# damaggu/StableKeypoints

Measured on AMD Instinct MI355X. Metric: images/sec (token-opt step, 512², N=500 tokens), higher is better.
Workload: dtype f32

## Files before the change

### include/skp.h

```cpp
#ifndef SKP_H
#define SKP_H

#ifdef __cplusplus
extern "C" {
#endif

#define SKP_OK 0
#define SKP_EBADARG (-1)
#define SKP_ELAUNCH (-2)
#define SKP_MAX_LAYERS 16

const char* skp_last_error(void);
int skp_version(void);

int skp_capture_fwd(const float* z_low, int BH, int s, int N, int R, float* attn, float* stats, void* stream);

int skp_capture_bwd(const float* z_low, int BH, int s, int N, int R, const float* dattn, int group, long long sb,
                    long long sp, long long sn, float gscale, const float* stats, float* dz_low, float* workspace,
                    void* stream);

int skp_capture_maps_fwd(const float* const* z_low, const int* sizes, int L, int B, int H, int N, int R, float* maps,
                         float* const* stats, void* stream);

int skp_capture_maps_bwd(const float* const* z_low, const int* sizes, int L, int B, int H, int N, int R,
// ... 133 lines not shown
int skp_wino2_weights(const float* w, int K, int C, int flip, float* U, void* stream);
int skp_conv3x3_wino2(const float* x, const float* U, const float* bias, const float* residual, float* y, int B,
                      int C, int K, int H, int W, int nsplit, float* ws, void* stream);
int skp_conv3x3_wino2_gn(const float* x, const float* U, const float* bias, const float* residual, float* y, int B,
                         int C, int K, int H, int W, int nsplit, float* ws, float* gn_part, void* stream);
int skp_wino2_vtransform(const float* x, float* V, int B, int C, int H, int W, void* stream);
int skp_wino2_vtransform_gn(const float* x, const float* stats, const float* gamma, const float* beta,
                            const float* shift, int G, int act, float* V, int B, int C, int H, int W, void* stream);
int skp_conv3x3_wino2_v(const float* V, const float* U, const float* bias, const float* residual, float* y, int B,
                        int C, int K, int H, int W, int nsplit, float* ws, void* stream);
int skp_conv3x3_wino2_v_gn(const float* V, const float* U, const float* bias, const float* residual, float* y, int B,
                           int C, int K, int H, int W, int nsplit, float* ws, float* gn_part, void* stream);
int skp_wino2s2_weights(const float* w, int K, int C, float* U, void* stream);
int skp_conv3x3s2_f2(const float* x, const float* U, const float* bias, float* y, int B, int C, int K, int H, int W,
                     int nsplit, float* ws, void* stream);

int skp_map_range(const float* maps, int n, int h, int w, float* range, void* stream);
int skp_render_sheet(const float* images, int n, int H, int W, const float* maps, int h, int w, const float* range,
                     const float* lut, float alpha, const float* points, int K, float radius,
                     const unsigned char* colors, int rows, int cols, int f, int pad, unsigned char* out,
                     void* stream);

int skp_tta_reduce_workspace(int B, int n, int S);
int skp_tta_reduce(const float* maps, int B, int C, int n, int S, const float* theta_inv, float* pos, float* avg,
                   void* workspace, void* stream);

#ifdef __cplusplus
}
#endif
#endif
// ... 1 lines not shown
```

### stablekeypoints_amd/_lib.py

```python
import ctypes
import os

import torch

_HERE = os.path.dirname(os.path.abspath(__file__))
LIB_PATH = os.environ.get("SKP_LIB", os.path.join(_HERE, "libskp.so"))

_c_int, _c_float, _c_ll, _p = ctypes.c_int, ctypes.c_float, ctypes.c_longlong, ctypes.c_void_p

_SIGS = {
    "skp_capture_fwd": [_p, _c_int, _c_int, _c_int, _c_int, _p, _p, _p],
    "skp_capture_bwd": [_p, _c_int, _c_int, _c_int, _c_int, _p, _c_int, _c_ll, _c_ll, _c_ll, _c_float, _p, _p, _p,
                        _p],
    "skp_capture_maps_fwd": [ctypes.POINTER(_p), ctypes.POINTER(_c_int), _c_int, _c_int, _c_int, _c_int, _c_int, _p,
                             ctypes.POINTER(_p), _p],
    "skp_capture_maps_bwd": [ctypes.POINTER(_p), ctypes.POINTER(_c_int), _c_int, _c_int, _c_int, _c_int, _c_int, _p,
                             _c_float, ctypes.POINTER(_p), ctypes.POINTER(_p), _p, _p],
    "skp_capture_maps_bwd_sel": [ctypes.POINTER(_p), ctypes.POINTER(_c_int), _c_int, _c_int, _c_int, _c_int, _c_int,
                                 _p, _c_int, _p, _c_float, ctypes.POINTER(_p), ctypes.POINTER(_p), _p, _p],
    "skp_sel_bwd_timing": [_c_int],
    "skp_sel_bwd_timing_read": [_p, _p],
    "skp_capture_maps_bwd_sel_workspace": [ctypes.POINTER(_c_int), _c_int, _c_int, _c_int, _c_int, _c_int, _c_int],
    "skp_aggregate": [ctypes.POINTER(_p), _c_int, _c_int, _c_int, _c_int, _p, _c_int, _p, _p],
    "skp_resize_bilinear": [_p, _c_int, _c_int, _c_int, _p, _p],
# ... 52 lines not shown
    "skp_wino_weights": [_p, _c_int, _c_int, _c_int, _p, _p],
    "skp_conv3x3_wino": [_p, _p, _p, _p, _p, _c_int, _c_int, _c_int, _c_int, _c_int, _c_int, _p, _p],
    "skp_wino2_weights": [_p, _c_int, _c_int, _c_int, _p, _p],
    "skp_conv3x3_wino2": [_p, _p, _p, _p, _p, _c_int, _c_int, _c_int, _c_int, _c_int, _c_int, _p, _p],
    "skp_conv3x3_wino2_gn": [_p, _p, _p, _p, _p, _c_int, _c_int, _c_int, _c_int, _c_int, _c_int, _p, _p, _p],
    "skp_groupnorm_fwd_part": [_p, _p, _p, _p, _p, _c_int, _c_int, _c_int, _c_ll, _c_int, _c_float, _c_int, _p, _p, _p,
                               _p],
    "skp_groupnorm_stats": [_p, _p, _c_int, _c_int, _c_ll, _c_int, _c_float, _p, _p, _p],
    "skp_groupnorm_stats_part": [_p, _c_int, _p, _c_int, _c_int, _c_ll, _c_int, _c_float, _p, _p, _p],
    "skp_wino2_vtransform": [_p, _p, _c_int, _c_int, _c_int, _c_int, _p],
    "skp_wino2_vtransform_gn": [_p, _p, _p, _p, _p, _c_int, _c_int, _p, _c_int, _c_int, _c_int, _c_int, _p],
    "skp_conv3x3_wino2_v": [_p, _p, _p, _p, _p, _c_int, _c_int, _c_int, _c_int, _c_int, _c_int, _p, _p],
    "skp_conv3x3_wino2_v_gn": [_p, _p, _p, _p, _p, _c_int, _c_int, _c_int, _c_int, _c_int, _c_int, _p, _p, _p],
    "skp_wino2s2_weights": [_p, _c_int, _c_int, _p, _p],
    "skp_conv3x3s2_f2":   [_p, _p, _p, _p, _c_int, _c_int, _c_int, _c_int, _c_int, _c_int, _p, _p],
    "skp_map_range": [_p, _c_int, _c_int, _c_int, _p, _p],
    "skp_render_sheet": [_p, _c_int, _c_int, _c_int, _p, _c_int, _c_int, _p, _p, _c_float, _p, _c_int, _c_float, _p,
                         _c_int, _c_int, _c_int, _c_int, _p, _p],
    "skp_tta_reduce_workspace": [_c_int, _c_int, _c_int],
    "skp_tta_reduce": [_p, _c_int, _c_int, _c_int, _c_int, _p, _p, _p, _p, _p],
    "skp_version": [],
}


_RESTYPE = {"skp_capture_maps_bwd_sel_workspace": _c_ll}
_MEASUREMENT_ONLY = {"skp_sel_bwd_timing", "skp_sel_bwd_timing_read"}


class SkpLibraryError(RuntimeError):
    pass


_lib = None


def lib():
    global _lib
    if _lib is None:
        if not os.path.exists(LIB_PATH):
            raise SkpLibraryError(f"libskp.so not found at {LIB_PATH}: build it with "
                                  "`python -c 'import __graft_entry__ as g; g.build()'` or `make -C stablekeypoints_amd/csrc`")
# ... 41 lines not shown
```

### stablekeypoints_amd/csrc/skp_conv.hip

```cpp
#include <cstdlib>

#include "skp_common.h"
#include "skp_gn.h"

using namespace skp;

#ifndef SKP_WINO_DEBUG
#define SKP_WINO_DEBUG 0
#endif
#ifndef SKP_WINO2_DEBUG
#define SKP_WINO2_DEBUG 0
#endif

namespace {

typedef float f32x4 __attribute__((ext_vector_type(4)));
typedef unsigned int u32x4 __attribute__((ext_vector_type(4)));

constexpr int kMT = 64;
constexpr int kNC = 32;
constexpr int kCK = 4;
constexpr int kP = 36;
constexpr int kThreads = 512;
constexpr int kUs = kCK * kNC * kP;
// ... 625 lines not shown
    case 9: W2_VMCNT(9); break;
    case 10: W2_VMCNT(10); break;
    case 11: W2_VMCNT(11); break;
    case 12: W2_VMCNT(12); break;
    case 13: W2_VMCNT(13); break;
    case 14: W2_VMCNT(14); break;
    case 15: W2_VMCNT(15); break;
    default: W2_VMCNT(0); break;
  }
}

#ifndef SKP_W2_RS4
#define SKP_W2_RS4 0
#endif

template <int EPI, int HH, int TXB, int NW, bool VST = false, bool S2 = false>
__device__ __forceinline__ void wino2_body(const W2Smem& sm, const float* __restrict__ x, const float* __restrict__ U,
                                           const float* __restrict__ bias, const float* __restrict__ res,
                                           float* __restrict__ y, int C, int K, int H, int W, int img, int x0,
                                           int y0, int kb, int c0, int csplit, int wv, int dbg,
                                           float2* __restrict__ gnp) {
  using Geo = w2::GeoT<TXB, NW>;
  constexpr int kChF = Geo::CHF, kRowF = Geo::RF, kRawInstr = Geo::RAW_INSTR, NI = Geo::NI, RR = Geo::RR,
                RC = Geo::RC;
  static_assert(!S2 || (TXB == 8 && NW == 4 && !VST && (EPI & ~1) == 0), "stride-2 form: half-height blocks, bias only");
  constexpr int kUP = S2 ? w2::kUP2 : w2::kUP, kUF = S2 ? w2::kUF2 : w2::kUF, kUInstr = kUF / 256;
  constexpr int NP = S2 ? (HH ? 10 : 15) : 18;
  constexpr int kInstr = kRawInstr + kUInstr;
  constexpr int kMaxRaw = (kRawInstr + NW - 1) / NW;
  constexpr int kMaxU = (kUInstr + NW - 1) / NW + 1;
  constexpr int NT = NW * WAVE;
// ... 196 lines not shown
      }
    }

  }

  W2_VMCNT(0);
  __syncthreads();
  if (dbg & 32) return;
  if constexpr (S2) {
    constexpr int PLS2 = 8 * 16 + 4;
    static_assert(16 * PLS2 <= Geo::RAWF, "stride-2 exchange planes fit one raw slot");
    const int Ho = H / 2, Wo = W / 2;
    float* pl = R0 + (lane & 15) * PLS2 + 2 * (2 * wm + (lane >> 5)) * 16 + 8 * ((lane >> 4) & 1);
#pragma unroll
    for (int blk = 0; blk < 2; ++blk) {
      float o[4][4];
#pragma unroll
      for (int r = 0; r < 4; ++r) {
        float m[NP];
#pragma unroll
        for (int q = 0; q < NP; ++q) m[q] = acc[blk][q][r];
        w2::s2_output<HH>(m, o[r]);
      }
      if (HH != blk) {
#pragma unroll
        for (int f = 0; f < 2; ++f)
#pragma unroll
          for (int h = 0; h < 2; ++h)
            *reinterpret_cast<float4*>(pl + f * 16 + 4 * h) =
                make_float4(o[2 * h][2 * f], o[2 * h][2 * f + 1], o[2 * h + 1][2 * f], o[2 * h + 1][2 * f + 1]);
      }
      __syncthreads();
      if (HH == blk) {
#pragma unroll
        for (int f = 0; f < 2; ++f)
#pragma unroll
          for (int h = 0; h < 2; ++h) {
            float4* d = reinterpret_cast<float4*>(pl + f * 16 + 4 * h);
            const float4 p = *d;
            *d = make_float4(o[2 * h][2 * f] + p.x, o[2 * h][2 * f + 1] + p.y, o[2 * h + 1][2 * f] + p.z,
                             o[2 * h + 1][2 * f + 1] + p.w);
          }
      }
      __syncthreads();
#pragma unroll
      for (int i = 0; i < 16 * 32 / NT; ++i) {
        const int idx = i * NT + tid;
        const int c = idx >> 5, row = (idx >> 2) & 7, c4 = idx & 3;
        const float4 p = *reinterpret_cast<const float4*>(R0 + c * PLS2 + row * 16 + 4 * c4);
        const int k = kb * w2::kNC + 16 * blk + c;
        const float bv = (EPI & 1) ? bias[k] : 0.0f;
        const size_t o4 = (((size_t)img * K + k) * Ho + y0 / 2 + row) * Wo + x0 / 2 + 4 * c4;
        const float4 v = make_float4(p.x + bv, p.y + bv, p.z + bv, p.w + bv);
        if (dbg & 128) __builtin_nontemporal_store(f32x4{v.x, v.y, v.z, v.w}, reinterpret_cast<f32x4*>(y + o4));
        else if (!(dbg & 64)) *reinterpret_cast<float4*>(y + o4) = v;
      }
      if (blk == 0) __syncthreads();
    }
  } else {
    constexpr int PH = (TXB == 8 && NW == 4) ? 16 : 32;
    constexpr int PLS = (TXB == 8 ? PH * 32 : NI * 256) + 4;
    float* const P2 = RS == 2 ? U1 : R2;
    auto plane_of = [&](int c) -> float* {
      float* b = (c >> 2) == 0 ? R0 : (c >> 2) == 1 ? R1 : (c >> 2) == 2 ? P2 : U0;
      return b + (c & 3) * PLS + (c >> 2) * 16;
    };
    float* pl = plane_of(lane & 15);
    const int pbase = TXB == 8 ? (4 * (2 * wm + (lane >> 5))) * 32 + 4 * (4 * ((lane >> 4) & 1))
                               : wm * 256 + (4 * (lane >> 4)) * 16;
    constexpr int PW = TXB == 8 ? 32 : 16;
#pragma unroll
    for (int blk = 0; blk < 2; ++blk) {
      if (HH != blk) {
#pragma unroll
        for (int r = 0; r < 4; ++r) {
          float m[18], o[16];
#pragma unroll
          for (int q = 0; q < 18; ++q) m[q] = acc[blk][q][r];
          w2::half_output<HH>(m, o);
#pragma unroll
          for (int f = 0; f < 4; ++f)
            *reinterpret_cast<float4*>(pl + pbase + f * PW + 4 * r) =
                make_float4(o[4 * f], o[4 * f + 1], o[4 * f + 2], o[4 * f + 3]);
        }
      }
      __syncthreads();
      if (HH == blk) {
#pragma unroll
        for (int r = 0; r < 4; ++r) {
          float m[18], o[16];
#pragma unroll
          for (int q = 0; q < 18; ++q) m[q] = acc[blk][q][r];
          w2::half_output<HH>(m, o);
#pragma unroll
          for (int f = 0; f < 4; ++f) {
            float4* d = reinterpret_cast<float4*>(pl + pbase + f * PW + 4 * r);
            const float4 p = *d;
            *d = make_float4(o[4 * f] + p.x, o[4 * f + 1] + p.y, o[4 * f + 2] + p.z, o[4 * f + 3] + p.w);
          }
        }
      }
      __syncthreads();
      constexpr int PCF = TXB == 8 ? PH * 8 : NI * 64;
      constexpr int NIT = 16 * PCF / NT;
      static_assert(TXB != 8 || NIT == 8, "TXB 8: eight wave instructions per wave");
      float g1[4] = {0.f, 0.f, 0.f, 0.f}, g2[4] = {0.f, 0.f, 0.f, 0.f}, piv[4] = {0.f, 0.f, 0.f, 0.f};
#pragma unroll
      for (int i = 0; i < NIT; ++i) {
        const int idx = TXB == 8 ? (((tid >> 6) * NIT + i) << 6) + (tid & 63) : i * NT + tid;
        const int c = idx / PCF, q = idx % PCF;
        const float4 v0 = *reinterpret_cast<const float4*>(plane_of(c) + 4 * q);
        const int k = kb * w2::kNC + 16 * blk + c;
        const float bv = (EPI & 1) ? bias[k] : 0.0f;
        size_t o;
        if (TXB == 8) {
          const int row = q >> 3, c4 = q & 7;
          o = (((size_t)img * K + k) * H + y0 + row) * W + x0 + 4 * c4;
        } else {
          o = ((size_t)(img + (q >> 6)) * K + k) * 256 + 4 * (q & 63);
        }
        float4 v = make_float4(v0.x + bv, v0.y + bv, v0.z + bv, v0.w + bv);
        if (EPI & 2) {
          const float4 rv = *reinterpret_cast<const float4*>(res + o);
          v.x += rv.x;
          v.y += rv.y;
          v.z += rv.z;
          v.w += rv.w;
        }
        if (dbg & 128) __builtin_nontemporal_store(f32x4{v.x, v.y, v.z, v.w}, reinterpret_cast<f32x4*>(y + o));
        else if (!(dbg & 64)) *reinterpret_cast<float4*>(y + o) = v;
        if (TXB == 8 && gnp) {
          if ((i & 1) == 0) piv[i >> 1] = __builtin_bit_cast(float, __builtin_amdgcn_readfirstlane(__builtin_bit_cast(int, v.x)));
          const float p = piv[i >> 1];
          const float dx = v.x - p, dy = v.y - p, dz = v.z - p, dw = v.w - p;
          g1[i >> 1] += (dx + dy) + (dz + dw);
          g2[i >> 1] += (dx * dx + dy * dy) + (dz * dz + dw * dw);
        }
      }
// ... 25 lines not shown
          const int J = (tid >> 6) * NIT + 2 * r;
          const int c = (J << 6) / PCF, piece = ((J << 6) % PCF) >> 6;
          const int k = kb * w2::kNC + 16 * blk + c;
          const int seg = ((y0 + 8 * piece) >> 4) * (W >> 5) + (x0 >> 5);
          const float p = r == 0 ? piv[0] : r == 1 ? piv[1] : r == 2 ? piv[2] : piv[3];
          constexpr float inv_n = 1.0f / 512.0f;
          gnp[((size_t)img * K + k) * (size_t)((H >> 4) * (W >> 5)) + seg] =
              make_float2(p + x * inv_n, fmaxf(x2 - x * (x * inv_n), 0.0f));
        }
      }
      if (blk == 0) __syncthreads();
    }
  }
}

template <int EPI, int TXB, int NW = 8, bool S2 = false>
__global__ __launch_bounds__(NW * WAVE) __attribute__((amdgpu_waves_per_eu(2, 2))) void wino2_kernel(
    const float* __restrict__ x, const float* __restrict__ U, const float* __restrict__ bias,
    const float* __restrict__ res, float* __restrict__ y, int nimg, int C, int K, int H, int W, int bw, int bpi,
    int nblk, int nkb, int kb_major, int csplit, int dbg, float2* __restrict__ gnp) {
  __shared__ __attribute__((aligned(16))) float R0[w2::GeoT<TXB, NW>::RAWF], R1[w2::GeoT<TXB, NW>::RAWF],
      R2[(TXB == 4 && NW == 4) ? 4 : w2::GeoT<TXB, NW>::RAWF],
      R3[(TXB == 8 && NW == 8 && SKP_W2_RS4) ? w2::GeoT<TXB, NW>::RAWF : 4];
  constexpr int UF = S2 ? w2::kUF2 : w2::kUF;
  __shared__ __attribute__((aligned(16))) float U0[UF], U1[UF], U2[NW == 4 ? 4 : UF];
  const int G = gridDim.x;
  const int g = blockIdx.x;
  const int Lg = (G % 8 == 0) ? (g % 8) * (G / 8) + g / 8 : g;
  const int sp = Lg / (nblk * nkb);
  const int L = Lg - sp * (nblk * nkb);
  y += (size_t)sp * nimg * K * (S2 ? (H / 2) * (W / 2) : H * W);
  int tb, kb;
  if (kb_major) {
    kb = L / nblk;
    tb = L - kb * nblk;
  } else {
    tb = L / nkb;
    kb = L - tb * nkb;
  }
  int img, x0 = 0, y0 = 0;
  if (TXB == 8) {
    img = tb / bpi;
    const int br = tb - img * bpi;
    const int by = br / bw;
    x0 = 32 * (br - by * bw);
    y0 = (NW == 4 ? 16 : 32) * by;
  } else {
    img = (NW == 4 ? 2 : 4) * tb;
  }
  const int wv = __builtin_amdgcn_readfirstlane(threadIdx.x >> 6);
  const W2Smem sm{R0, R1, R2, R3, U0, U1, U2};
  const int c0 = sp * csplit;
  if (wv < NW / 2)
    wino2_body<EPI, 0, TXB, NW, false, S2>(sm, x, U, bias, res, y, C, K, H, W, img, x0, y0, kb, c0, csplit, wv, dbg, gnp);
  else wino2_body<EPI, 1, TXB, NW, false, S2>(sm, x, U, bias, res, y, C, K, H, W, img, x0, y0, kb, c0, csplit, wv, dbg, gnp);
}

__global__ void wino2_weights_kernel(const float* __restrict__ w, int K, int C, int flip, float* __restrict__ U) {
  const long long i = blockIdx.x * (long long)blockDim.x + threadIdx.x;
  if (i >= (long long)K * C) return;
  const int k = (int)(i / C), c = (int)(i - (long long)k * C);
  double g[9];
  for (int u = 0; u < 3; ++u)
    for (int v = 0; v < 3; ++v)
      g[3 * u + v] = flip ? (double)w[((size_t)c * K + k) * 9 + (2 - u) * 3 + (2 - v)]
                          : (double)w[((size_t)k * C + c) * 9 + u * 3 + v];
  const double Gm[6][3] = {{1.0, 0.0, 0.0},
                           {1.0 / 3, 1.0 / 3, 1.0 / 3},
                           {-1.0 / 3, 1.0 / 3, -1.0 / 3},
                           {-16.0 / 15, -8.0 / 15, -4.0 / 15},
// ... 18 lines not shown
  double g[9];
  for (int u = 0; u < 9; ++u) g[u] = (double)w[((size_t)k * C + c) * 9 + u];
  const double Gm[5][3] = {{1.0, 0.0, 0.0}, {1.0, 0.0, 1.0}, {0.0, 0.0, 1.0}, {0.0, 1.0, 0.0}, {0.0, 1.0, 0.0}};
  double t[5][3];
  for (int a = 0; a < 5; ++a)
    for (int v = 0; v < 3; ++v) t[a][v] = Gm[a][0] * g[v] + Gm[a][1] * g[3 + v] + Gm[a][2] * g[6 + v];
  float* out = U + (((size_t)(k / w2::kNC) * C + c) * w2::kNC + (k % w2::kNC)) * w2::kUP2;
  for (int p = 0; p < w2::kUP2; ++p) out[p] = 0.0f;
  for (int a = 0; a < 5; ++a)
    for (int b = 0; b < 5; ++b) {
      const int p = 5 * a + b;
      out[p < 15 ? p : p + 1] = (float)(t[a][0] * Gm[b][0] + t[a][1] * Gm[b][1] + t[a][2] * Gm[b][2]);
    }
}

template <int EPI>
__global__ __launch_bounds__(4 * WAVE) __attribute__((amdgpu_waves_per_eu(2, 2))) void wino2v_kernel(
    const float* __restrict__ V, const float* __restrict__ U, const float* __restrict__ bias,
    const float* __restrict__ res, float* __restrict__ y, int nimg, int C, int K, int H, int W, int bw, int bpi,
    int nblk, int nkb, int kb_major, int csplit, int dbg, float2* __restrict__ gnp) {
  __shared__ __attribute__((aligned(16))) float U0[w2::kUF], U1[w2::kUF], U2[w2::kUF];
  static_assert(3 * w2::kUF * 4 <= 80 * 1024, "two workgroups per CU");
  static_assert(4 * (16 * 32 + 4) + 48 <= w2::kUF / 2, "a plane buffer per half U slot");
  const int G = gridDim.x;
  const int g = blockIdx.x;
  const int Lg = (G % 8 == 0) ? (g % 8) * (G / 8) + g / 8 : g;
  const int sp = Lg / (nblk * nkb);
  const int L = Lg - sp * (nblk * nkb);
  y += (size_t)sp * nimg * K * H * W;
  int tb, kb;
  if (kb_major) {
    kb = L / nblk;
    tb = L - kb * nblk;
  } else {
    tb = L / nkb;
    kb = L - tb * nkb;
  }
  const int img = tb / bpi;
  const int br = tb - img * bpi;
  const int by = br / bw;
  const int x0 = 32 * (br - by * bw), y0 = 16 * by;
  const int wv = __builtin_amdgcn_readfirstlane(threadIdx.x >> 6);
  const W2Smem sm{U0 + w2::kUF / 2, U1 + w2::kUF / 2, nullptr, nullptr, U0, U1, U2};
  const int c0 = sp * csplit;
  if (wv < 2)
    wino2_body<EPI, 0, 8, 4, true>(sm, V, U, bias, res, y, C, K, H, W, img, x0, y0, kb, c0, csplit, wv, dbg, gnp);
  else wino2_body<EPI, 1, 8, 4, true>(sm, V, U, bias, res, y, C, K, H, W, img, x0, y0, kb, c0, csplit, wv, dbg, gnp);
}

template <int GN>
__global__ __launch_bounds__(4 * WAVE) void wino2_vtransform_kernel(
    const float* __restrict__ x, const float* __restrict__ stats, const float* __restrict__ gamma,
    const float* __restrict__ beta, const float* __restrict__ shift, int G, float* __restrict__ V, int C, int H, int W,
    int bw, int bpi) {
  using Geo = w2::GeoT<8, 4>;
  constexpr int RR = Geo::RR, RC = Geo::RC, kChF = Geo::CHF, kRowF = Geo::RF;
  __shared__ __attribute__((aligned(16))) float R[Geo::RAWF];
  const int tid = threadIdx.x, lane = tid & 63;
  const int nst = C / w2::kCK;
  const int tb = blockIdx.x / nst, st = blockIdx.x - tb * nst;
  const int img = tb / bpi;
  const int br = tb - img * bpi;
// ... 50 lines not shown
  SKP_CHECK_ARG(w && U, "null pointer");
  SKP_CHECK_ARG(K > 0 && C > 0, "non-positive shape");
  SKP_CHECK_ARG(K % w2::kNC == 0, "output channels must be a multiple of 32");
  const long long n = (long long)K * C;
  hipLaunchKernelGGL(wino2s2_weights_kernel, dim3((unsigned)((n + 255) / 256)), dim3(256), 0, as_stream(stream), w, K,
                     C, U);
  SKP_LAUNCH_CHECK();
  return SKP_OK;
}

namespace {
int wino_nt_flag(long long out_bytes, int nsplit) {
  if (nsplit > 1) return 0;
  return out_bytes >= (256LL << 20) ? 128 : 0;
}
}

extern "C" int skp_conv3x3s2_f2(const float* x, const float* U, const float* bias, float* y, int B, int C, int K,
                                int H, int W, int nsplit, float* ws, void* stream) {
  SKP_CHECK_ARG(x && U && y, "null pointer");
  SKP_CHECK_ARG(B > 0 && C > 0 && K > 0 && H > 0 && W > 0, "non-positive shape");
  SKP_CHECK_ARG(C % w2::kCK == 0, "input channels must be a multiple of 4");
  SKP_CHECK_ARG(K % w2::kNC == 0, "output channels must be a multiple of 32");
  SKP_CHECK_ARG(H % 32 == 0 && W % 32 == 0, "H and W must be multiples of 32");
  SKP_CHECK_ARG(nsplit >= 1 && C % (w2::kCK * nsplit) == 0, "nsplit must divide C into multiples of 4");
  SKP_CHECK_ARG(nsplit == 1 || ws, "split-K needs a workspace of nsplit·B·K·(H/2)·(W/2) floats");
  SKP_CHECK_ARG(aligned16(x) && aligned16(U) && aligned16(y) && (!ws || aligned16(ws)), "tensors must be 16-byte aligned");
  SKP_CHECK_ARG((long long)B * C * H * W * 4 < 0x7fffffffLL, "input larger than 2 GiB (32-bit buffer offsets)");
  const int bw = W / 32, bpi = (H / 16) * bw;
  const long long nblk = (long long)B * bpi;
  const int nkb = K / w2::kNC;
  SKP_CHECK_ARG(nblk * nkb * nsplit <= 0x7fffffffLL, "grid too large");
  float* out = nsplit > 1 ? ws : y;
  hipStream_t st = as_stream(stream);
  const dim3 grid((unsigned)(nblk * nkb * nsplit));
  const int fl = SKP_WINO2_DEBUG | wino_nt_flag((long long)B * K * (H / 2) * (W / 2) * 4, nsplit);
  if (nsplit == 1 && bias)
    hipLaunchKernelGGL((wino2_kernel<1, 8, 4, true>), grid, dim3(4 * WAVE), 0, st, x, U, bias, nullptr, out, B, C, K, H,
                       W, bw, bpi, (int)nblk, nkb, 0, C / nsplit, fl, nullptr);
  else
    hipLaunchKernelGGL((wino2_kernel<0, 8, 4, true>), grid, dim3(4 * WAVE), 0, st, x, U, nullptr, nullptr, out, B, C, K,
                       H, W, bw, bpi, (int)nblk, nkb, 0, C / nsplit, fl, nullptr);
  SKP_LAUNCH_CHECK();
  if (nsplit > 1) return splitk_reduce(ws, nsplit, B, K, (H / 2) * (W / 2), bias, nullptr, y, st);
  return SKP_OK;
}

extern "C" int skp_conv3x3_wino2_gn(const float* x, const float* U, const float* bias, const float* residual, float* y,
                                    int B, int C, int K, int H, int W, int nsplit, float* ws, float* gn_part,
                                    void* stream) {
  SKP_CHECK_ARG(x && U && y, "null pointer");
  SKP_CHECK_ARG(!gn_part || (nsplit == 1 && H % 32 == 0 && W % 32 == 0 && (reinterpret_cast<uintptr_t>(gn_part) & 7) == 0),
                "gn_part: one split, H and W multiples of 32, 8-byte aligned");
  SKP_CHECK_ARG(B > 0 && C > 0 && K > 0 && H > 0 && W > 0, "non-positive shape");
  SKP_CHECK_ARG(C % w2::kCK == 0, "input channels must be a multiple of 4");
  SKP_CHECK_ARG(K % w2::kNC == 0, "output channels must be a multiple of 32");
  const bool g16 = H == 16 && W == 16;
// ... 2 lines not shown
  SKP_CHECK_ARG(nsplit >= 1 && C % (w2::kCK * nsplit) == 0, "nsplit must divide C into multiples of 4");
  SKP_CHECK_ARG(nsplit == 1 || ws, "split-K needs a workspace of nsplit·B·K·H·W floats");
  SKP_CHECK_ARG(aligned16(x) && aligned16(U) && aligned16(y) && (!residual || aligned16(residual)) &&
                    (!ws || aligned16(ws)),
                "tensors must be 16-byte aligned");
  SKP_CHECK_ARG((long long)B * C * H * W * 4 < 0x7fffffffLL, "input larger than 2 GiB (32-bit buffer offsets)");
  const int bw = W / 32, bpi = (H / 16) * bw;
  const long long nblk = g16 ? B / 2 : (long long)B * bpi;
  const int nkb = K / w2::kNC;
  SKP_CHECK_ARG(nblk * nkb * nsplit <= 0x7fffffffLL, "grid too large");
  const int dbg = SKP_WINO2_DEBUG;
  const int kb_major = 0;
  const int epi = nsplit > 1 ? 0 : (bias ? 1 : 0) | (residual ? 2 : 0);
  float* out = nsplit > 1 ? ws : y;
  hipStream_t st = as_stream(stream);
  const dim3 grid((unsigned)(nblk * nkb * nsplit));
  const int fl = dbg | wino_nt_flag((long long)B * K * H * W * 4, nsplit);
  float2* gnp = reinterpret_cast<float2*>(gn_part);
#define SKP_WG2(E)                                                                                            \
  if (g16)                                                                                                    \
    hipLaunchKernelGGL((wino2_kernel<E, 4, 4>), grid, dim3(4 * WAVE), 0, st, x, U, bias, residual, out, B, C, K,  \
                       H, W, bw, bpi, (int)nblk, nkb, kb_major, C / nsplit, fl, nullptr);                              \
  else                                                                                                        \
    hipLaunchKernelGGL((wino2_kernel<E, 8, 4>), grid, dim3(4 * WAVE), 0, st, x, U, bias, residual, out, B, C, K,  \
                       H, W, bw, bpi, (int)nblk, nkb, kb_major, C / nsplit, fl, gnp)
  switch (epi) {
    case 0: SKP_WG2(0); break;
    case 1: SKP_WG2(1); break;
    case 2: SKP_WG2(2); break;
    default: SKP_WG2(3); break;
  }
#undef SKP_WG2
  SKP_LAUNCH_CHECK();
  if (nsplit > 1) return splitk_reduce(ws, nsplit, B, K, H * W, bias, residual, y, st);
  return SKP_OK;
}

extern "C" int skp_conv3x3_wino2(const float* x, const float* U, const float* bias, const float* residual, float* y,
                                 int B, int C, int K, int H, int W, int nsplit, float* ws, void* stream) {
  return skp_conv3x3_wino2_gn(x, U, bias, residual, y, B, C, K, H, W, nsplit, ws, nullptr, stream);
// ... 51 lines not shown
  SKP_CHECK_ARG(K % w2::kNC == 0, "output channels must be a multiple of 32");
  SKP_CHECK_ARG(H % 32 == 0 && W % 32 == 0, "H and W must be multiples of 32");
  SKP_CHECK_ARG(nsplit >= 1 && C % (w2::kCK * nsplit) == 0, "nsplit must divide C into multiples of 4");
  SKP_CHECK_ARG(nsplit == 1 || ws, "split-K needs a workspace of nsplit·B·K·H·W floats");
  SKP_CHECK_ARG(aligned16(V) && aligned16(U) && aligned16(y) && (!residual || aligned16(residual)) &&
                    (!ws || aligned16(ws)),
                "tensors must be 16-byte aligned");
  const int bw = W / 32, bpi = (H / 16) * bw;
  const long long nblk = (long long)B * bpi;
  const int nkb = K / w2::kNC;
  SKP_CHECK_ARG(nblk * nkb * nsplit <= 0x7fffffffLL, "grid too large");
  const int kb_major = 0;
  const int epi = nsplit > 1 ? 0 : (bias ? 1 : 0) | (residual ? 2 : 0);
  float* out = nsplit > 1 ? ws : y;
  hipStream_t st = as_stream(stream);
  const dim3 grid((unsigned)(nblk * nkb * nsplit));
  const int fl = SKP_WINO2_DEBUG | wino_nt_flag((long long)B * K * H * W * 4, nsplit);
  float2* gnp = reinterpret_cast<float2*>(gn_part);
#define SKP_WV(E)                                                                                                  \
  hipLaunchKernelGGL((wino2v_kernel<E>), grid, dim3(4 * WAVE), 0, st, V, U, bias, residual, out, B, C, K, H, W, bw, \
                     bpi, (int)nblk, nkb, kb_major, C / nsplit, fl, gnp)
  switch (epi) {
    case 0: SKP_WV(0); break;
    case 1: SKP_WV(1); break;
    case 2: SKP_WV(2); break;
    default: SKP_WV(3); break;
  }
#undef SKP_WV
  SKP_LAUNCH_CHECK();
  if (nsplit > 1) return splitk_reduce(ws, nsplit, B, K, H * W, bias, residual, y, st);
  return SKP_OK;
}

extern "C" int skp_conv3x3_wino2_v(const float* V, const float* U, const float* bias, const float* residual, float* y,
                                   int B, int C, int K, int H, int W, int nsplit, float* ws, void* stream) {
  return skp_conv3x3_wino2_v_gn(V, U, bias, residual, y, B, C, K, H, W, nsplit, ws, nullptr, stream);
// ... 2 lines not shown
```

### stablekeypoints_amd/ops.py

```python
import ctypes
import os

import torch

from . import _lib
from ._lib import call, ptr, stream

F32 = torch.float32

_TIMER = None


def set_kernel_timer(timer):
    global _TIMER
    _TIMER = timer


class _NoTimer:
    def __enter__(self):
        return self

    def __exit__(self, *a):
        return False

# ... 1451 lines not shown
    bmax = max(1, (2 ** 31 - 1) // per_img)
    gnp = None
    if gn and GN_EPI and H % 32 == 0 and W % 32 == 0 and all(
            _wino_plan(min(B, b0 + bmax) - b0, C, K, H, W)[:2] == (True, 1) for b0 in range(0, B, bmax)):
        nseg = (H // 16) * (W // 32)
        gnp = torch.empty(B, K, nseg, 2, device=x.device, dtype=F32)
    for b0 in range(0, B, bmax):
        b1 = min(B, b0 + bmax)
        _wino_launch(x[b0:b1], weight, flip, bias, None if residual is None else residual[b0:b1], y[b0:b1], K,
                     None if gnp is None else gnp[b0:b1])
    if gnp is not None:
        y._skp_gn = (y._version, gnp, gnp.shape[2])
    return y


def _wino_launch(x, weight, flip, bias, residual, y, K, gnp=None):
    B, C, H, W = x.shape
    v2, nsplit, _ = _wino_plan(B, C, K, H, W)
    U = _wino_u(weight, flip, v2)
    ws = torch.empty(nsplit, B, K, H, W, device=x.device, dtype=F32) if nsplit > 1 else None
    name = "skp_conv3x3_wino2" if v2 else "skp_conv3x3_wino"
    args = (ptr(x), ptr(U), ptr(bias) if bias is not None else None,
            ptr(residual) if residual is not None else None, ptr(y), B, C, K, H, W, nsplit,
            ptr(ws) if ws is not None else None)
    with _timed(name, 0):
        if gnp is not None:
            call("skp_conv3x3_wino2_gn", *args, ptr(gnp), stream(x.device))
        else:
            call(name, *args, stream(x.device))


class Conv3x3(torch.autograd.Function):
# ... 71 lines not shown
def conv3x3_s2(x, weight, bias=None):
    _lib.require_device(x)
    if not conv3x3_s2_eligible(x, weight):
        raise ValueError(f"conv3x3_s2: unsupported x {tuple(x.shape)} / weight {tuple(weight.shape)}")
    x = _c16(x)
    B, C, H, W = x.shape
    K = weight.shape[0]
    y = torch.empty(B, K, H // 2, W // 2, device=x.device, dtype=F32)
    U = _wino_u(weight, False, "s2")
    b = None if bias is None else _c(bias.detach())
    bmax = max(1, (2 ** 31 - 1) // (C * H * W * 4))
    for b0 in range(0, B, bmax):
        b1 = min(B, b0 + bmax)
        _, nsplit, _ = _wino_plan(b1 - b0, C, K, H, W)
        ws = torch.empty(nsplit, b1 - b0, K, H // 2, W // 2, device=x.device, dtype=F32) if nsplit > 1 else None
        with _timed("skp_conv3x3s2_f2", 0):
            call("skp_conv3x3s2_f2", ptr(x[b0:b1]), ptr(U), ptr(b), ptr(y[b0:b1]), b1 - b0, C, K, H, W, nsplit,
                 ptr(ws), stream(x.device))
    return y


def conv3x3(x, weight, bias=None, residual=None):
    _lib.require_device(x)
    if weight.requires_grad:
        raise ValueError("conv3x3: the weight must be frozen (requires_grad=False)")
    B, C, H, W = x.shape
    K = weight.shape[0]
    if tuple(weight.shape[1:]) != (C, 3, 3):
        raise ValueError(f"conv3x3: weight {tuple(weight.shape)} does not fit input {tuple(x.shape)}")
    if residual is not None and tuple(residual.shape) != (B, K, H, W):
# ... 48 lines not shown
        call("skp_groupnorm_stats_part", ptr(pre[0]), pre[1], ptr(shift), B, C, H * W, int(groups), float(eps),
             ptr(stats), ptr(part), stream(dev))
    else:
        call("skp_groupnorm_stats", ptr(x), ptr(shift), B, C, H * W, int(groups), float(eps), ptr(stats), ptr(part),
             stream(dev))
    V = torch.empty(B * C * (H // 4) * (W // 4) * 36, device=dev, dtype=F32)
    with _timed("skp_wino2_vtransform_gn", 0):
        call("skp_wino2_vtransform_gn", ptr(x), ptr(stats), ptr(g), ptr(b), ptr(shift), int(groups), int(bool(act)),
             ptr(V), B, C, H, W, stream(dev))
    _, nsplit, _ = _wino_plan(B, C, K, H, W)
    U = _wino_u(weight, False, True)
    y = torch.empty(B, K, H, W, device=dev, dtype=F32)
    ws = torch.empty(nsplit, B, K, H, W, device=dev, dtype=F32) if nsplit > 1 else None
    gnp = torch.empty(B, K, (H // 16) * (W // 32), 2, device=dev, dtype=F32) if GN_EPI and nsplit == 1 else None
    bias = None if bias is None else _c(bias.detach())
    with _timed("skp_conv3x3_wino2_v", 0):
        call("skp_conv3x3_wino2_v_gn", ptr(V), ptr(U), ptr(bias), ptr(residual), ptr(y), B, C, K, H, W, nsplit,
             ptr(ws), ptr(gnp), stream(dev))
    if gnp is not None:
        y._skp_gn = (y._version, gnp, gnp.shape[2])
    return y


TAB10 = ((31, 119, 180), (255, 127, 14), (44, 160, 44), (214, 39, 40), (148, 103, 189), (140, 86, 75),
         (227, 119, 194), (127, 127, 127), (188, 189, 34), (23, 190, 207))
_VIRIDIS_ANCHORS = ((0, (0.267004, 0.004874, 0.329415)), (32, (0.278826, 0.175490, 0.483397)),
                    (64, (0.229739, 0.322361, 0.545706)), (96, (0.172719, 0.448791, 0.557885)),
                    (128, (0.127568, 0.566949, 0.550556)), (160, (0.157851, 0.683765, 0.501686)),
                    (192, (0.369214, 0.788888, 0.382914)), (224, (0.678489, 0.863742, 0.189503)),
                    (255, (0.993248, 0.906157, 0.143936)))
# ... 125 lines not shown
```

Before: 44.15.

## Add optional persistent job loop to Winograd kernels and prefetch epilogue operands

Adds a persistent-grid mode to the wino2 and wino2v kernels, where each workgroup loops over several tile jobs separated by a barrier. The grid size comes from an occupancy query or a user setting. The epilogue now loads bias and residual values into registers before the final tile transform and barrier, so those global loads overlap with compute. The persistent mode is off by default (auto table all false), so by default only the prefetch path runs. It costs extra register pressure and adds a ctypes call before every conv launch.

```diff
diff --git a/include/skp.h b/include/skp.h
--- a/include/skp.h
+++ b/include/skp.h
@@ -171,6 +171,7 @@
 int skp_wino2s2_weights(const float* w, int K, int C, float* U, void* stream);
 int skp_conv3x3s2_f2(const float* x, const float* U, const float* bias, float* y, int B, int C, int K, int H, int W,
                      int nsplit, float* ws, void* stream);
+int skp_wino2_persistent(int n);
 
 int skp_map_range(const float* maps, int n, int h, int w, float* range, void* stream);
 int skp_render_sheet(const float* images, int n, int H, int W, const float* maps, int h, int w, const float* range,
diff --git a/stablekeypoints_amd/_lib.py b/stablekeypoints_amd/_lib.py
--- a/stablekeypoints_amd/_lib.py
+++ b/stablekeypoints_amd/_lib.py
@@ -90,6 +90,7 @@
     "skp_conv3x3_wino2_v_gn": [_p, _p, _p, _p, _p, _c_int, _c_int, _c_int, _c_int, _c_int, _c_int, _p, _p, _p],
     "skp_wino2s2_weights": [_p, _c_int, _c_int, _p, _p],
     "skp_conv3x3s2_f2":   [_p, _p, _p, _p, _c_int, _c_int, _c_int, _c_int, _c_int, _c_int, _p, _p],
+    "skp_wino2_persistent": [_c_int],
     "skp_map_range": [_p, _c_int, _c_int, _c_int, _p, _p],
     "skp_render_sheet": [_p, _c_int, _c_int, _c_int, _p, _c_int, _c_int, _p, _p, _c_float, _p, _c_int, _c_float, _p,
                          _c_int, _c_int, _c_int, _c_int, _p, _p],
@@ -100,7 +101,7 @@
 
 
 _RESTYPE = {"skp_capture_maps_bwd_sel_workspace": _c_ll}
-_MEASUREMENT_ONLY = {"skp_sel_bwd_timing", "skp_sel_bwd_timing_read"}
+_MEASUREMENT_ONLY = {"skp_sel_bwd_timing", "skp_sel_bwd_timing_read", "skp_wino2_persistent"}
 
 
 class SkpLibraryError(RuntimeError):
diff --git a/stablekeypoints_amd/csrc/skp_conv.hip b/stablekeypoints_amd/csrc/skp_conv.hip
--- a/stablekeypoints_amd/csrc/skp_conv.hip
+++ b/stablekeypoints_amd/csrc/skp_conv.hip
@@ -1,3 +1,4 @@
+#include <atomic>
 #include <cstdlib>
 
 #include "skp_common.h"
@@ -663,7 +664,7 @@
 #define SKP_W2_RS4 0
 #endif
 
-template <int EPI, int HH, int TXB, int NW, bool VST = false, bool S2 = false>
+template <int EPI, int HH, int TXB, int NW, bool VST = false, bool S2 = false, bool PERS = false>
 __device__ __forceinline__ void wino2_body(const W2Smem& sm, const float* __restrict__ x, const float* __restrict__ U,
                                            const float* __restrict__ bias, const float* __restrict__ res,
                                            float* __restrict__ y, int C, int K, int H, int W, int img, int x0,
@@ -890,6 +891,10 @@
     float* pl = R0 + (lane & 15) * PLS2 + 2 * (2 * wm + (lane >> 5)) * 16 + 8 * ((lane >> 4) & 1);
 #pragma unroll
     for (int blk = 0; blk < 2; ++blk) {
+      float bvs[16 * 32 / NT];
+#pragma unroll
+      for (int i = 0; i < 16 * 32 / NT; ++i)
+        bvs[i] = (EPI & 1) ? bias[kb * w2::kNC + 16 * blk + ((i * NT + tid) >> 5)] : 0.0f;
       float o[4][4];
 #pragma unroll
       for (int r = 0; r < 4; ++r) {
@@ -918,6 +923,10 @@
                              o[2 * h + 1][2 * f + 1] + p.w);
           }
       }
+      if (EPI & 1) {
+#pragma unroll
+        for (int i = 0; i < 16 * 32 / NT; ++i) asm volatile("" ::"v"(bvs[i]));
+      }
       __syncthreads();
 #pragma unroll
       for (int i = 0; i < 16 * 32 / NT; ++i) {
@@ -925,7 +934,7 @@
         const int c = idx >> 5, row = (idx >> 2) & 7, c4 = idx & 3;
         const float4 p = *reinterpret_cast<const float4*>(R0 + c * PLS2 + row * 16 + 4 * c4);
         const int k = kb * w2::kNC + 16 * blk + c;
-        const float bv = (EPI & 1) ? bias[k] : 0.0f;
+        const float bv = bvs[i];
         const size_t o4 = (((size_t)img * K + k) * Ho + y0 / 2 + row) * Wo + x0 / 2 + 4 * c4;
         const float4 v = make_float4(p.x + bv, p.y + bv, p.z + bv, p.w + bv);
         if (dbg & 128) __builtin_nontemporal_store(f32x4{v.x, v.y, v.z, v.w}, reinterpret_cast<f32x4*>(y + o4));
@@ -945,8 +954,34 @@
     const int pbase = TXB == 8 ? (4 * (2 * wm + (lane >> 5))) * 32 + 4 * (4 * ((lane >> 4) & 1))
                                : wm * 256 + (4 * (lane >> 4)) * 16;
     constexpr int PW = TXB == 8 ? 32 : 16;
+    constexpr int PCF = TXB == 8 ? PH * 8 : NI * 64;
+    constexpr int NIT = 16 * PCF / NT;
+    static_assert(TXB != 8 || NIT == 8, "TXB 8: eight wave instructions per wave");
+    constexpr bool PRE = TXB == 8 && NW == 4;
 #pragma unroll
     for (int blk = 0; blk < 2; ++blk) {
+      auto elem = [&](int i, int& c, int& q, int& k) -> size_t {
+        const int idx = TXB == 8 ? (((tid >> 6) * NIT + i) << 6) + (tid & 63) : i * NT + tid;
+        c = idx / PCF;
+        q = idx % PCF;
+        k = kb * w2::kNC + 16 * blk + c;
+        if (TXB == 8) {
+          const int row = q >> 3, c4 = q & 7;
+          return (((size_t)img * K + k) * H + y0 + row) * W + x0 + 4 * c4;
+        }
+        return ((size_t)(img + (q >> 6)) * K + k) * 256 + 4 * (q & 63);
+      };
+      float bvs[NIT];
+      float4 rvs[NIT];
+      if (PRE && (EPI & 3)) {
+#pragma unroll
+        for (int i = 0; i < NIT; ++i) {
+          int c, q, k;
+          const size_t o = elem(i, c, q, k);
+          bvs[i] = (EPI & 1) ? bias[k] : 0.0f;
+          if (EPI & 2) rvs[i] = *reinterpret_cast<const float4*>(res + o);
+        }
+      }
       if (HH != blk) {
 #pragma unroll
         for (int r = 0; r < 4; ++r) {
@@ -976,28 +1011,24 @@
           }
         }
       }
+      if (PRE && (EPI & 3)) {
+#pragma unroll
+        for (int i = 0; i < NIT; ++i) {
+          if (EPI & 1) asm volatile("" ::"v"(bvs[i]));
+          if (EPI & 2) asm volatile("" ::"v"(rvs[i].x), "v"(rvs[i].y), "v"(rvs[i].z), "v"(rvs[i].w));
+        }
+      }
       __syncthreads();
-      constexpr int PCF = TXB == 8 ? PH * 8 : NI * 64;
-      constexpr int NIT = 16 * PCF / NT;
-      static_assert(TXB != 8 || NIT == 8, "TXB 8: eight wave instructions per wave");
       float g1[4] = {0.f, 0.f, 0.f, 0.f}, g2[4] = {0.f, 0.f, 0.f, 0.f}, piv[4] = {0.f, 0.f, 0.f, 0.f};
 #pragma unroll
       for (int i = 0; i < NIT; ++i) {
-        const int idx = TXB == 8 ? (((tid >> 6) * NIT + i) << 6) + (tid & 63) : i * NT + tid;
-        const int c = idx / PCF, q = idx % PCF;
+        int c, q, k;
+        const size_t o = elem(i, c, q, k);
         const float4 v0 = *reinterpret_cast<const float4*>(plane_of(c) + 4 * q);
-        const int k = kb * w2::kNC + 16 * blk + c;
-        const float bv = (EPI & 1) ? bias[k] : 0.0f;
-        size_t o;
-        if (TXB == 8) {
-          const int row = q >> 3, c4 = q & 7;
-          o = (((size_t)img * K + k) * H + y0 + row) * W + x0 + 4 * c4;
-        } else {
-          o = ((size_t)(img + (q >> 6)) * K + k) * 256 + 4 * (q & 63);
-        }
+        const float bv = !(EPI & 1) ? 0.0f : PRE ? bvs[i] : bias[k];
         float4 v = make_float4(v0.x + bv, v0.y + bv, v0.z + bv, v0.w + bv);
         if (EPI & 2) {
-          const float4 rv = *reinterpret_cast<const float4*>(res + o);
+          const float4 rv = PRE ? rvs[i] : *reinterpret_cast<const float4*>(res + o);
           v.x += rv.x;
           v.y += rv.y;
           v.z += rv.z;
@@ -1053,46 +1084,62 @@
   }
 }
 
-template <int EPI, int TXB, int NW = 8, bool S2 = false>
+__device__ __forceinline__ void wino2_job_end() {
+  asm volatile("" ::: "memory");
+  __builtin_amdgcn_s_waitcnt(0xC07F);
+  __builtin_amdgcn_s_barrier();
+  asm volatile("" ::: "memory");
+}
+
+template <int EPI, int TXB, int NW = 8, bool S2 = false, bool PERS = false>
 __global__ __launch_bounds__(NW * WAVE) __attribute__((amdgpu_waves_per_eu(2, 2))) void wino2_kernel(
     const float* __restrict__ x, const float* __restrict__ U, const float* __restrict__ bias,
-    const float* __restrict__ res, float* __restrict__ y, int nimg, int C, int K, int H, int W, int bw, int bpi,
-    int nblk, int nkb, int kb_major, int csplit, int dbg, float2* __restrict__ gnp) {
+    const float* __restrict__ res, float* __restrict__ yout, int nimg, int C, int K, int H, int W, int bw, int bpi,
+    int nblk, int nkb, int kb_major, int csplit, int dbg, float2* __restrict__ gnp, int njobs) {
+  static_assert(!PERS || (TXB == 8 && NW == 4), "job loop: half-height blocks of 4 waves");
   __shared__ __attribute__((aligned(16))) float R0[w2::GeoT<TXB, NW>::RAWF], R1[w2::GeoT<TXB, NW>::RAWF],
       R2[(TXB == 4 && NW == 4) ? 4 : w2::GeoT<TXB, NW>::RAWF],
       R3[(TXB == 8 && NW == 8 && SKP_W2_RS4) ? w2::GeoT<TXB, NW>::RAWF : 4];
   constexpr int UF = S2 ? w2::kUF2 : w2::kUF;
   __shared__ __attribute__((aligned(16))) float U0[UF], U1[UF], U2[NW == 4 ? 4 : UF];
-  const int G = gridDim.x;
-  const int g = blockIdx.x;
-  const int Lg = (G % 8 == 0) ? (g % 8) * (G / 8) + g / 8 : g;
-  const int sp = Lg / (nblk * nkb);
-  const int L = Lg - sp * (nblk * nkb);
-  y += (size_t)sp * nimg * K * (S2 ? (H / 2) * (W / 2) : H * W);
-  int tb, kb;
-  if (kb_major) {
-    kb = L / nblk;
-    tb = L - kb * nblk;
-  } else {
-    tb = L / nkb;
-    kb = L - tb * nkb;
-  }
-  int img, x0 = 0, y0 = 0;
-  if (TXB == 8) {
-    img = tb / bpi;
-    const int br = tb - img * bpi;
-    const int by = br / bw;
-    x0 = 32 * (br - by * bw);
-    y0 = (NW == 4 ? 16 : 32) * by;
-  } else {
-    img = (NW == 4 ? 2 : 4) * tb;
-  }
   const int wv = __builtin_amdgcn_readfirstlane(threadIdx.x >> 6);
   const W2Smem sm{R0, R1, R2, R3, U0, U1, U2};
-  const int c0 = sp * csplit;
-  if (wv < NW / 2)
-    wino2_body<EPI, 0, TXB, NW, false, S2>(sm, x, U, bias, res, y, C, K, H, W, img, x0, y0, kb, c0, csplit, wv, dbg, gnp);
-  else wino2_body<EPI, 1, TXB, NW, false, S2>(sm, x, U, bias, res, y, C, K, H, W, img, x0, y0, kb, c0, csplit, wv, dbg, gnp);
+  const int G = PERS ? njobs : (int)gridDim.x;
+  long long gl = blockIdx.x;
+  if (PERS && gl >= njobs) return;
+  for (;;) {
+    const int g = (int)gl;
+    const int Lg = (G % 8 == 0) ? (g % 8) * (G / 8) + g / 8 : g;
+    const int sp = Lg / (nblk * nkb);
+    const int L = Lg - sp * (nblk * nkb);
+    float* y = yout + (size_t)sp * nimg * K * (S2 ? (H / 2) * (W / 2) : H * W);
+    int tb, kb;
+    if (kb_major) {
+      kb = L / nblk;
+      tb = L - kb * nblk;
+    } else {
+      tb = L / nkb;
+      kb = L - tb * nkb;
+    }
+    int img, x0 = 0, y0 = 0;
+    if (TXB == 8) {
+      img = tb / bpi;
+      const int br = tb - img * bpi;
+      const int by = br / bw;
+      x0 = 32 * (br - by * bw);
+      y0 = (NW == 4 ? 16 : 32) * by;
+    } else {
+      img = (NW == 4 ? 2 : 4) * tb;
+    }
+    const int c0 = sp * csplit;
+    if (wv < NW / 2)
+      wino2_body<EPI, 0, TXB, NW, false, S2, PERS>(sm, x, U, bias, res, y, C, K, H, W, img, x0, y0, kb, c0, csplit, wv, dbg, gnp);
+    else wino2_body<EPI, 1, TXB, NW, false, S2, PERS>(sm, x, U, bias, res, y, C, K, H, W, img, x0, y0, kb, c0, csplit, wv, dbg, gnp);
+    if (!PERS) break;
+    gl += gridDim.x;
+    if (gl >= njobs) break;
+    wino2_job_end();
+  }
 }
 
 __global__ void wino2_weights_kernel(const float* __restrict__ w, int K, int C, int flip, float* __restrict__ U) {
@@ -1141,38 +1188,46 @@
     }
 }
 
-template <int EPI>
+template <int EPI, bool PERS = false>
 __global__ __launch_bounds__(4 * WAVE) __attribute__((amdgpu_waves_per_eu(2, 2))) void wino2v_kernel(
     const float* __restrict__ V, const float* __restrict__ U, const float* __restrict__ bias,
-    const float* __restrict__ res, float* __restrict__ y, int nimg, int C, int K, int H, int W, int bw, int bpi,
-    int nblk, int nkb, int kb_major, int csplit, int dbg, float2* __restrict__ gnp) {
+    const float* __restrict__ res, float* __restrict__ yout, int nimg, int C, int K, int H, int W, int bw, int bpi,
+    int nblk, int nkb, int kb_major, int csplit, int dbg, float2* __restrict__ gnp, int njobs) {
   __shared__ __attribute__((aligned(16))) float U0[w2::kUF], U1[w2::kUF], U2[w2::kUF];
   static_assert(3 * w2::kUF * 4 <= 80 * 1024, "two workgroups per CU");
   static_assert(4 * (16 * 32 + 4) + 48 <= w2::kUF / 2, "a plane buffer per half U slot");
-  const int G = gridDim.x;
-  const int g = blockIdx.x;
-  const int Lg = (G % 8 == 0) ? (g % 8) * (G / 8) + g / 8 : g;
-  const int sp = Lg / (nblk * nkb);
-  const int L = Lg - sp * (nblk * nkb);
-  y += (size_t)sp * nimg * K * H * W;
-  int tb, kb;
-  if (kb_major) {
-    kb = L / nblk;
-    tb = L - kb * nblk;
-  } else {
-    tb = L / nkb;
-    kb = L - tb * nkb;
-  }
-  const int img = tb / bpi;
-  const int br = tb - img * bpi;
-  const int by = br / bw;
-  const int x0 = 32 * (br - by * bw), y0 = 16 * by;
   const int wv = __builtin_amdgcn_readfirstlane(threadIdx.x >> 6);
   const W2Smem sm{U0 + w2::kUF / 2, U1 + w2::kUF / 2, nullptr, nullptr, U0, U1, U2};
-  const int c0 = sp * csplit;
-  if (wv < 2)
-    wino2_body<EPI, 0, 8, 4, true>(sm, V, U, bias, res, y, C, K, H, W, img, x0, y0, kb, c0, csplit, wv, dbg, gnp);
-  else wino2_body<EPI, 1, 8, 4, true>(sm, V, U, bias, res, y, C, K, H, W, img, x0, y0, kb, c0, csplit, wv, dbg, gnp);
+  const int G = PERS ? njobs : (int)gridDim.x;
+  long long gl = blockIdx.x;
+  if (PERS && gl >= njobs) return;
+  for (;;) {
+    const int g = (int)gl;
+    const int Lg = (G % 8 == 0) ? (g % 8) * (G / 8) + g / 8 : g;
+    const int sp = Lg / (nblk * nkb);
+    const int L = Lg - sp * (nblk * nkb);
+    float* y = yout + (size_t)sp * nimg * K * H * W;
+    int tb, kb;
+    if (kb_major) {
+      kb = L / nblk;
+      tb = L - kb * nblk;
+    } else {
+      tb = L / nkb;
+      kb = L - tb * nkb;
+    }
+    const int img = tb / bpi;
+    const int br = tb - img * bpi;
+    const int by = br / bw;
+    const int x0 = 32 * (br - by * bw), y0 = 16 * by;
+    const int c0 = sp * csplit;
+    if (wv < 2)
+      wino2_body<EPI, 0, 8, 4, true, false, PERS>(sm, V, U, bias, res, y, C, K, H, W, img, x0, y0, kb, c0, csplit, wv, dbg, gnp);
+    else wino2_body<EPI, 1, 8, 4, true, false, PERS>(sm, V, U, bias, res, y, C, K, H, W, img, x0, y0, kb, c0, csplit, wv, dbg, gnp);
+    if (!PERS) break;
+    gl += gridDim.x;
+    if (gl >= njobs) break;
+    wino2_job_end();
+  }
 }
 
 template <int GN>
@@ -1253,6 +1308,44 @@
   if (nsplit > 1) return 0;
   return out_bytes >= (256LL << 20) ? 128 : 0;
 }
+
+std::atomic<int> g_wino2_persistent{-1};
+enum Wino2Family { kFamConv = 0, kFamV = 1, kFamS2 = 2 };
+constexpr bool kWino2PersistAuto[3] = {false, false, false};
+
+int wino2_resident(const void* kern, std::atomic<int>* cache) {
+  int dev = 0;
+  if (hipGetDevice(&dev) != hipSuccess || dev < 0 || dev >= 64) return 0;
+  int r = cache[dev].load(std::memory_order_relaxed);
+  if (r > 0) return r;
+  int per_cu = 0, ncu = 0;
+  if (hipOccupancyMaxActiveBlocksPerMultiprocessor(&per_cu, kern, 4 * WAVE, 0) != hipSuccess ||
+      hipDeviceGetAttribute(&ncu, hipDeviceAttributeMultiprocessorCount, dev) != hipSuccess || per_cu <= 0 || ncu <= 0)
+    return 0;
+  r = per_cu * ncu;
+  if (r >= 8) r -= r % 8;
+  cache[dev].store(r, std::memory_order_relaxed);
+  return r;
+}
+
+int wino2_persistent_grid(Wino2Family fam, long long jobs, const void* kern) {
+  static std::atomic<int> cache[3][64];
+  const int mode = g_wino2_persistent.load(std::memory_order_relaxed);
+  if (mode == 0 || (mode < 0 && !kWino2PersistAuto[fam])) return 0;
+  if (mode > 0) return mode;
+  const int r = wino2_resident(kern, cache[fam]);
+  if (r <= 0) return -1;
+  return jobs > r ? r : 0;
+}
+}
+
+extern "C" int skp_wino2_persistent(int n) {
+  const int prev = g_wino2_persistent.load(std::memory_order_relaxed);
+  if (n < -1) {
+    ::skp::set_error("skp_wino2_persistent: n must be -1 (automatic), 0 (one job per workgroup) or a workgroup count");
+    return prev;
+  }
+  return g_wino2_persistent.exchange(n, std::memory_order_relaxed);
 }
 
 extern "C" int skp_conv3x3s2_f2(const float* x, const float* U, const float* bias, float* y, int B, int C, int K,
@@ -1272,14 +1365,22 @@
   SKP_CHECK_ARG(nblk * nkb * nsplit <= 0x7fffffffLL, "grid too large");
   float* out = nsplit > 1 ? ws : y;
   hipStream_t st = as_stream(stream);
-  const dim3 grid((unsigned)(nblk * nkb * nsplit));
+  const int njobs = (int)(nblk * nkb * nsplit);
+  const int pg = wino2_persistent_grid(kFamS2, njobs, reinterpret_cast<const void*>(&wino2_kernel<1, 8, 4, true, true>));
+  SKP_CHECK_ARG(pg >= 0, "occupancy query failed");
+  const dim3 grid((unsigned)(pg ? pg : njobs));
   const int fl = SKP_WINO2_DEBUG | wino_nt_flag((long long)B * K * (H / 2) * (W / 2) * 4, nsplit);
-  if (nsplit == 1 && bias)
-    hipLaunchKernelGGL((wino2_kernel<1, 8, 4, true>), grid, dim3(4 * WAVE), 0, st, x, U, bias, nullptr, out, B, C, K, H,
-                       W, bw, bpi, (int)nblk, nkb, 0, C / nsplit, fl, nullptr);
-  else
-    hipLaunchKernelGGL((wino2_kernel<0, 8, 4, true>), grid, dim3(4 * WAVE), 0, st, x, U, nullptr, nullptr, out, B, C, K,
-                       H, W, bw, bpi, (int)nblk, nkb, 0, C / nsplit, fl, nullptr);
+#define SKP_WS2(E, P, BIAS)                                                                                          \
+  hipLaunchKernelGGL((wino2_kernel<E, 8, 4, true, P>), grid, dim3(4 * WAVE), 0, st, x, U, BIAS, nullptr, out, B, C, K, \
+                     H, W, bw, bpi, (int)nblk, nkb, 0, C / nsplit, fl, nullptr, njobs)
+  if (nsplit == 1 && bias) {
+    if (pg) SKP_WS2(1, true, bias);
+    else SKP_WS2(1, false, bias);
+  } else {
+    if (pg) SKP_WS2(0, true, nullptr);
+    else SKP_WS2(0, false, nullptr);
+  }
+#undef SKP_WS2
   SKP_LAUNCH_CHECK();
   if (nsplit > 1) return splitk_reduce(ws, nsplit, B, K, (H / 2) * (W / 2), bias, nullptr, y, st);
   return SKP_OK;
@@ -1312,16 +1413,23 @@
   const int epi = nsplit > 1 ? 0 : (bias ? 1 : 0) | (residual ? 2 : 0);
   float* out = nsplit > 1 ? ws : y;
   hipStream_t st = as_stream(stream);
-  const dim3 grid((unsigned)(nblk * nkb * nsplit));
+  const int njobs = (int)(nblk * nkb * nsplit);
+  const int pg =
+      g16 ? 0 : wino2_persistent_grid(kFamConv, njobs, reinterpret_cast<const void*>(&wino2_kernel<3, 8, 4, false, true>));
+  SKP_CHECK_ARG(pg >= 0, "occupancy query failed");
+  const dim3 grid((unsigned)(pg ? pg : njobs));
   const int fl = dbg | wino_nt_flag((long long)B * K * H * W * 4, nsplit);
   float2* gnp = reinterpret_cast<float2*>(gn_part);
 #define SKP_WG2(E)                                                                                            \
   if (g16)                                                                                                    \
     hipLaunchKernelGGL((wino2_kernel<E, 4, 4>), grid, dim3(4 * WAVE), 0, st, x, U, bias, residual, out, B, C, K,  \
-                       H, W, bw, bpi, (int)nblk, nkb, kb_major, C / nsplit, fl, nullptr);                              \
+                       H, W, bw, bpi, (int)nblk, nkb, kb_major, C / nsplit, fl, nullptr, njobs);                       \
+  else if (pg)                                                                                                \
+    hipLaunchKernelGGL((wino2_kernel<E, 8, 4, false, true>), grid, dim3(4 * WAVE), 0, st, x, U, bias, residual, out, B, \
+                       C, K, H, W, bw, bpi, (int)nblk, nkb, kb_major, C / nsplit, fl, gnp, njobs);                     \
   else                                                                                                        \
     hipLaunchKernelGGL((wino2_kernel<E, 8, 4>), grid, dim3(4 * WAVE), 0, st, x, U, bias, residual, out, B, C, K,  \
-                       H, W, bw, bpi, (int)nblk, nkb, kb_major, C / nsplit, fl, gnp)
+                       H, W, bw, bpi, (int)nblk, nkb, kb_major, C / nsplit, fl, gnp, njobs)
   switch (epi) {
     case 0: SKP_WG2(0); break;
     case 1: SKP_WG2(1); break;
@@ -1403,12 +1511,19 @@
   const int epi = nsplit > 1 ? 0 : (bias ? 1 : 0) | (residual ? 2 : 0);
   float* out = nsplit > 1 ? ws : y;
   hipStream_t st = as_stream(stream);
-  const dim3 grid((unsigned)(nblk * nkb * nsplit));
+  const int njobs = (int)(nblk * nkb * nsplit);
+  const int pg = wino2_persistent_grid(kFamV, njobs, reinterpret_cast<const void*>(&wino2v_kernel<3, true>));
+  SKP_CHECK_ARG(pg >= 0, "occupancy query failed");
+  const dim3 grid((unsigned)(pg ? pg : njobs));
   const int fl = SKP_WINO2_DEBUG | wino_nt_flag((long long)B * K * H * W * 4, nsplit);
   float2* gnp = reinterpret_cast<float2*>(gn_part);
-#define SKP_WV(E)                                                                                                  \
-  hipLaunchKernelGGL((wino2v_kernel<E>), grid, dim3(4 * WAVE), 0, st, V, U, bias, residual, out, B, C, K, H, W, bw, \
-                     bpi, (int)nblk, nkb, kb_major, C / nsplit, fl, gnp)
+#define SKP_WV(E)                                                                                                   \
+  if (pg)                                                                                                           \
+    hipLaunchKernelGGL((wino2v_kernel<E, true>), grid, dim3(4 * WAVE), 0, st, V, U, bias, residual, out, B, C, K, H, \
+                       W, bw, bpi, (int)nblk, nkb, kb_major, C / nsplit, fl, gnp, njobs);                            \
+  else                                                                                                              \
+    hipLaunchKernelGGL((wino2v_kernel<E>), grid, dim3(4 * WAVE), 0, st, V, U, bias, residual, out, B, C, K, H, W,   \
+                       bw, bpi, (int)nblk, nkb, kb_major, C / nsplit, fl, gnp, njobs)
   switch (epi) {
     case 0: SKP_WV(0); break;
     case 1: SKP_WV(1); break;
diff --git a/stablekeypoints_amd/ops.py b/stablekeypoints_amd/ops.py
--- a/stablekeypoints_amd/ops.py
+++ b/stablekeypoints_amd/ops.py
@@ -1489,8 +1489,18 @@
     return y
 
 
+WINO_PERSISTENT = -1
+
+
+def _wino_persistent_sync():
+    f = getattr(_lib.lib(), "skp_wino2_persistent", None)
+    if f is not None:
+        f(int(WINO_PERSISTENT))
+
+
 def _wino_launch(x, weight, flip, bias, residual, y, K, gnp=None):
     B, C, H, W = x.shape
+    _wino_persistent_sync()
     v2, nsplit, _ = _wino_plan(B, C, K, H, W)
     U = _wino_u(weight, flip, v2)
     ws = torch.empty(nsplit, B, K, H, W, device=x.device, dtype=F32) if nsplit > 1 else None
@@ -1592,6 +1602,7 @@
         b1 = min(B, b0 + bmax)
         _, nsplit, _ = _wino_plan(b1 - b0, C, K, H, W)
         ws = torch.empty(nsplit, b1 - b0, K, H // 2, W // 2, device=x.device, dtype=F32) if nsplit > 1 else None
+        _wino_persistent_sync()
         with _timed("skp_conv3x3s2_f2", 0):
             call("skp_conv3x3s2_f2", ptr(x[b0:b1]), ptr(U), ptr(b), ptr(y[b0:b1]), b1 - b0, C, K, H, W, nsplit,
                  ptr(ws), stream(x.device))
@@ -1670,6 +1681,7 @@
     ws = torch.empty(nsplit, B, K, H, W, device=dev, dtype=F32) if nsplit > 1 else None
     gnp = torch.empty(B, K, (H // 16) * (W // 32), 2, device=dev, dtype=F32) if GN_EPI and nsplit == 1 else None
     bias = None if bias is None else _c(bias.detach())
+    _wino_persistent_sync()
     with _timed("skp_conv3x3_wino2_v", 0):
         call("skp_conv3x3_wino2_v_gn", ptr(V), ptr(U), ptr(bias), ptr(residual), ptr(y), B, C, K, H, W, nsplit,
              ptr(ws), ptr(gnp), stream(dev))
```

New measurement: 44.18, median of 4. Within noise of the previous version (+0.1%).
